# TAMUparametric/PPOPT

Measured on AMD Instinct MI355X. Metric: candidate active-sets checked/sec (combinatorial mpQP), higher is better.
Workload: dtype f64

## Files before the change

ppopt_amd/csrc/batch_level.hip:

```cpp
#define MPC_GLOBAL __device__ __forceinline__
#define MPC_LB(...)
#include "batch_level.hpp"
#include "knobs.hpp"

#include <algorithm>
#include <cmath>
#include <cstdlib>
#include <cstring>
#include <mutex>
#include <tuple>
#include <vector>

namespace mpc {
namespace {

#define MEMBER const BatchMember &m = tab[blockIdx.y]
__device__ __forceinline__ int32_t *part_list_of(const BatchMember &m, int c) { return m.part_lists + (size_t)c * (size_t)m.n; }

__global__ void __launch_bounds__(256) m_zero(const BatchMember *__restrict__ tab) {
    MEMBER;
    for (int z = 0; z < m.n_zero; ++z) {
        const unsigned long long bytes = m.zero[z].bytes;
        if ((reinterpret_cast<unsigned long long>(m.zero[z].p) & 7ull) == 0 && (bytes & 7ull) == 0) {
            unsigned long long *p = reinterpret_cast<unsigned long long *>(m.zero[z].p);
            for (unsigned long long i = blockIdx.x * 256ull + threadIdx.x; i < bytes / 8; i += (unsigned long long)gridDim.x * 256ull) p[i] = 0ull;
        } else {
            unsigned char *p = reinterpret_cast<unsigned char *>(m.zero[z].p);
            for (unsigned long long i = blockIdx.x * 256ull + threadIdx.x; i < bytes; i += (unsigned long long)gridDim.x * 256ull) p[i] = 0;
        }
    }
}
__global__ void m_zero_counter(const BatchMember *__restrict__ tab, int which) {
    MEMBER;
    if (threadIdx.x == 0) { if (which == 0) m.ctr->work_retry = 0u; else m.ctr->work_region = 0u; }
}

template <int K, int NT, int SP>
__global__ void __launch_bounds__(256) m_kkt_thread(const BatchMember *__restrict__ tab) {
    MEMBER;
    k_kkt_thread<K, NT, SP>(m.pf, m.fr, m.n, m.kkt_code, m.kkt_L, m.status, m.targs, m.ctr);
}
__global__ void __launch_bounds__(1024) m_compact_small(const BatchMember *__restrict__ tab, int lo, int hi, int into_retry, int slot) {
    MEMBER;
    k_compact_small(m.status, (int)m.n, lo, hi, into_retry ? m.retry_list : m.theta_list, m.dcnt + slot);
}
template <int NT, int SLOTS>
__global__ void __launch_bounds__(64, (SLOTS >= 2 ? (NT <= 4 ? TH_WAVES_S2 : 2) : (NT >= 8 ? 3 : 4))) m_theta2(const BatchMember *__restrict__ tab) {
    MEMBER;
    ThetaArgs ta = m.targs;
    ta.chunk = 1;
    if (m.th_blocks > 0) { ta.wave_max = m.th_blocks; ta.wave_div = 0; }
    const uint8_t *kkc = nullptr;
    const double *kkl = nullptr;
    const int32_t *list = nullptr;
    if (m.use_kkt) { kkc = m.kkt_code; kkl = m.kkt_L; list = m.theta_list; ta.n_dev = m.dcnt + DC_THETA; }
    k_theta2<NT, SLOTS>(m.pf, m.fr, m.n, m.k, m.status, m.ctr, kkc, kkl, ta, list);
}
__global__ void __launch_bounds__(1024) m_partition_small(const BatchMember *__restrict__ tab, unsigned long long spec, int slot) {
    MEMBER;
    k_partition_small(m.status, (int)m.n, spec, m.part_lists, m.n, m.dcnt + slot);
}
__global__ void __launch_bounds__(64) m_verdict(const BatchMember *__restrict__ tab, int slot) {
    MEMBER;
    k_verdict(m.Pv, m.fr, m.n, m.k, m.status, m.ctr, part_list_of(m, 0), m.dcnt + slot);
}

__global__ void __launch_bounds__(64) m_recession(const BatchMember *__restrict__ tab) {
    MEMBER;
    if (!m.theta_open) return;
    k_recession(m.Pv, m.fr, m.n, m.k, m.status);
}

template <int NT, int SLOTS>
__global__ void __launch_bounds__(64, (SLOTS >= 2 ? 2 : R2W)) m_region2(const BatchMember *__restrict__ tab) {
    MEMBER;
    const uint8_t *kkc = m.use_kkt ? m.kkt_code : nullptr;
    const double *kkl = m.use_kkt ? m.kkt_L : nullptr;
    RegionStream rs = m.rs;
    rs.max_blocks = m.r2_blocks;
    if (m.r2_wcap > 0) rs.w_cap = m.r2_wcap;
    k_region2<NT, SLOTS>(m.pr, m.fr, m.k, part_list_of(m, 2), (int)m.n, m.status, m.headd, m.headi, m.fd, m.fi, m.epool, m.ctr, kkc, kkl, m.W,
                         m.kept_g, m.ldk, m.done_g, m.no_rbox ? (const double *)nullptr : m.targs.tvp + (size_t)NT * NT + NT, rs);
}

template <int MODE>
__global__ void __launch_bounds__(64) m_region_v1(const BatchMember *__restrict__ tab) {
    MEMBER;
    const int n_list = m.dcnt[DC_BATCH_RRETRY];
    if (n_list <= 0 || n_list > m.rcap) return;
    k_region<MODE>(m.Pr, m.fr, m.k, m.retry_list, n_list, m.status, m.recd, m.reci, m.rec_d, m.rec_i, m.ctr, m.facet_flags);
}

template <int SLOTS>
__global__ void __launch_bounds__(64, XQ_WAVES) m_xq(const BatchMember *__restrict__ tab) {
    MEMBER;
    DictCache dq = m.dc;
    dq.n_list_dev = m.dcnt + DC_OPEN;
    dq.max_blocks = m.xq_blocks;
    k_xq<SLOTS>(m.pf, m.fr, m.k, part_list_of(m, 3), (int)m.n, m.status, m.ctr, dq, m.nxc);
}
template <int NXC, int SLOTS>
__global__ void __launch_bounds__(64, (NXC * SLOTS >= 64 ? 2 : (NXC * SLOTS >= 32 ? X2_WAVES : X2_WAVES_16))) m_x2(const BatchMember *__restrict__ tab) {
    MEMBER;
    DictCache d = m.dc;
    d.n_list_dev = m.dcnt + (m.quick_test ? DC_OPEN_QT : DC_OPEN);
    d.max_blocks = m.x2_blocks;
    k_x2<NXC, SLOTS>(m.pf, m.fr, m.k, m.quick_test ? m.retry_list : part_list_of(m, 3), (int)m.n, m.status, m.ctr, d);
}

template <int MW>
__global__ void m_pruned_append(const BatchMember *__restrict__ tab) {
    MEMBER;
    k_pruned_append<MW>(m.fr, m.n, m.k, m.status, m.pruned + (size_t)m.n_pruned * MW, m.ctr, m.keep_lowdim);
}
// ... 209 lines not shown
```

ppopt_amd/csrc/kernels2.hpp:

```cpp
#pragma once
#include <type_traits>
#include "kernels.hpp"
#include "lp_reg.hpp"

namespace mpc {

constexpr double GROWTH_FRESH = 1e6;
#ifndef THETA_SCALE_MODE
#define THETA_SCALE_MODE 0
#endif
__device__ __forceinline__ double theta_row_scale(int ex) {
    if (THETA_SCALE_MODE == 1) return 1.0;
    if (THETA_SCALE_MODE == 2 && ex > 0) return 1.0;
    return ldexp(1.0, -ex);
}


struct ThetaArgs {
    const double *W, *UVp, *tvp, *tv_rows;
    int chunk;
    int cbuf_off;
    const int32_t *n_dev;
    const double *Wr, *UVrp, *AATr, *Me, *Ne, *gE;
    int ne;
// ... 204 lines not shown
            bbase[threadIdx.x] = tot ? atomicAdd(threadIdx.x == 0 ? ta.kt_n : ta.kx_n, tot) : 0;
        }
        __syncthreads();
        if (kind) {
            const int li = kind - 1;
            int pos = bbase[li] + __popcll((li ? m2 : m1) & ((1ull << lane) - 1ull));
            for (int w = 0; w < wave; ++w) pos += wcnt[li][w];
            (li ? ta.kx_list : ta.kt_list)[pos] = (int)c;
        }
    }
}

__device__ inline int kkt_fetch_or_solve(const DevProblem &P, int k, Smem &s, const uint8_t *kkcode, const double *Lin, size_t c,
                                         bool *ill = nullptr) {
    if (kkcode) {
        int code = kkcode[c];
        if (code != KK_UNDECIDED) {
            if (code == KK_ILL) { if (ill) *ill = true; code = 0; }
            if (code == 0) {
                const int cnt = k * (P.n_t + 1);
                const double *src = Lin + c * (size_t)cnt;
                for (int idx = lane_id(); idx < cnt; idx += 64) s.L[idx] = src[idx];
                wave_sync();
            }
            return code;
        }
    }
    return kkt_solve(P, k, s, ill);
}

#ifndef TH_WAVES_S2
#define TH_WAVES_S2 3
#endif
template <int NT, int SLOTS>
MPC_GLOBAL void MPC_LB(64, (SLOTS >= 2 ? (NT <= 4 ? TH_WAVES_S2 : 2) : (NT >= 8 ? 3 : 4))) k_theta2(const DevProblem *__restrict__ Pg, const int32_t *__restrict__ cands, long long n, int k,
                                                    uint8_t *__restrict__ status, LevelCounters *__restrict__ ctr,
                                                    const uint8_t *__restrict__ kkcode, const double *__restrict__ Lin, ThetaArgs ta,
                                                    const int32_t *__restrict__ list) {
    const DevProblem &P = *Pg;
    if (ta.n_dev) {
        n = *ta.n_dev;
        long long active = gridDim.x;
        if (ta.wave_max > 0) active = min(active, (long long)ta.wave_max);
        if (ta.wave_div > 0) active = min(active, max(256ll, n / ta.wave_div));
        if (ta.chunk <= 0) ta.chunk = (int)max(1ll, min(16ll, n / (active * 8)));
        if ((long long)blockIdx.x >= active || (long long)blockIdx.x * ta.chunk >= n) return;
    }
    extern __shared__ __attribute__((aligned(16))) double smem[];
    Smem s = carve(P, smem);
    constexpr int LS = NT + 1;
    const int lane = lane_id(), nt = P.n_t, nr = nt + 1, e = P.n_eq, nc = P.n_c, mode = P.kkt_mode, npre = P.n_tpre;
    double *tvm = s.T, *tvt = s.T + NT * NT, *blo = tvt + NT, *bhi = blo + NT, *Lp = s.T + NT * NT + 3 * NT;
    for (int idx = lane; idx < NT * NT + 3 * NT; idx += 64) s.T[idx] = ta.tvp[idx];
    wave_sync();
    unsigned long long pivots = 0, n_retry = 0;
    long long cyc_kkt = 0, cyc_theta = 0, cyc_rows = 0, cyc_s2 = 0;
    unsigned long long n_box1 = 0, n_box2 = 0;
    for (;;) {
        unsigned int c0 = 0;
        if (lane == 0) c0 = atomicAdd(&ctr->work_verdict, (unsigned)ta.chunk);
        c0 = (unsigned)__builtin_amdgcn_readfirstlane((int)c0);
        if (c0 >= n) break;
        const unsigned c1 = (unsigned)min((long long)c0 + ta.chunk, n);
      for (unsigned w = c0; w < c1; ++w) {
        const unsigned c = list ? (unsigned)list[w] : w;
        const int nin = load_active_set(P, cands + (size_t)c * k, k, s);
        int st = -1;
        const long long t0 = clock64();
        const int kk = kkt_fetch_or_solve(P, k, s, kkcode, Lin, c);
        const long long t1 = clock64();
        cyc_kkt += t1 - t0;
        bool singular = false, retry = false;
        if (kk == 1) st = ST_INFEASIBLE;
        else if (kk == 2) singular = true;
        else if (kk == 0) {
            for (int idx = lane; idx < k * LS; idx += 64) {
                const int a = idx / LS, t = idx - a * LS;
                Lp[idx] = t <= nt ? s.L[a * nr + t] : 0.0;
            }
            wave_sync();
            RegLp<NT + 2, SLOTS, true> lp;
            const int nlam = k - e, m = nlam + nin + npre;
            lp.m = m; lp.iters = 0; lp.max_iter = 50 * (m + nt) + 100; lp.growth = 0.0;
            lp.alive = (nt >= 31 ? 0xfffffffeu : ((1u << (nt + 1)) - 2u));
            lp.cv = nt + m + lane - 1;
            bool box_lam = false, box_slack = false;
            bool live[SLOTS];
#pragma unroll
            for (int sl = 0; sl < SLOTS; ++sl) live[sl] = (lane + 64 * sl) < (k - e) + nin + npre;
#pragma unroll
            for (int sl = 0; sl < SLOTS; ++sl) {
                const int i = lane + 64 * sl;
                double h = 0.0, g[NT];
#pragma unroll
                for (int t = 0; t < NT; ++t) g[t] = 0.0;
                lp.var[sl] = nt + i;
                lp.kind[sl] = i < nlam ? RK_PASSIVE : (i < m ? RK_INEQ : RK_DEAD);
                lp.w[sl] = 1.0; lp.winv[sl] = 1.0;
                bool pre = false;
                if (i < nlam) {
                    h = Lp[(e + i) * LS];
#pragma unroll
                    for (int t = 0; t < NT; ++t) g[t] = -Lp[(e + i) * LS + 1 + t];
                } else if (i < nlam + nin) {
                    const int ci = s.inact[i - nlam];
                    if (mode == 0) {
                        double acc[NT + 1], w[8];
                        const double *Wrow = ta.W + (size_t)ci * nc;
#pragma unroll
                        for (int a = 0; a < 8; ++a) { const int asv = s.as[a]; w[a] = Wrow[a < k ? asv : 0]; }
#pragma unroll
                        for (int t = 0; t <= NT; ++t) acc[t] = ta.UVp[ci * LS + t];
#pragma unroll
                        for (int a = 0; a < 8; ++a) {
// ... 103 lines not shown
                else if (r1 == LP_OPTIMAL && inf2) st = ST_FEASIBLE;
                else if (r1 == LP_OPTIMAL) {
#pragma unroll
                    for (int sl = 0; sl < S; ++sl) if (q.kind[sl] == RK_PASSIVE) q.kind[sl] = RK_INEQ;
                    const int r2 = q.phase1();
                    if (r2 == LP_ITERLIMIT) st = ST_LP_LIMIT;
                    else if (q.growth > GROWTH_FRESH) retry = true;
                    else st = r2 == LP_OPTIMAL ? ST_OPT_PENDING : ST_FEASIBLE;
                }
                lp_iters = q.iters;
            };
            bool compacted = false;
            if constexpr (SLOTS == 2) {
                const unsigned long long b0 = __ballot(live[0]), b1 = __ballot(live[1]);
                const int n_live = __popcll(b0) + __popcll(b1);
                if (ta.cbuf_off > 0 && n_live <= 64 && !inf1) {
                    constexpr int CS = NT + 4;
                    double *cb = smem + ta.cbuf_off;
                    int *cbi = reinterpret_cast<int *>(cb + 64 * CS);
                    const unsigned long long below = (1ull << lane) - 1ull;
#pragma unroll
                    for (int sl = 0; sl < 2; ++sl) {
                        if (live[sl]) {
                            const int pos = sl == 0 ? __popcll(b0 & below) : __popcll(b0) + __popcll(b1 & below);
#pragma unroll
                            for (int j = 0; j < NT + 2; ++j) cb[pos * CS + j] = lp.t[sl][j];
                            cb[pos * CS + NT + 2] = lp.w[sl];
                            cb[pos * CS + NT + 3] = lp.winv[sl];
                            cbi[2 * pos] = lp.var[sl];
                            cbi[2 * pos + 1] = lp.kind[sl];
                        }
                    }
                    wave_sync();
                    RegLp<NT + 2, 1, true> lp1;
                    lp1.m = n_live; lp1.iters = 0; lp1.max_iter = lp.max_iter; lp1.growth = 0.0;
                    lp1.alive = lp.alive; lp1.cv = lp.cv;
                    const bool has = lane < n_live;
#pragma unroll
                    for (int j = 0; j < NT + 2; ++j) lp1.t[0][j] = has ? cb[lane * CS + j] : 0.0;
                    lp1.w[0] = has ? cb[lane * CS + NT + 2] : 1.0;
                    lp1.winv[0] = has ? cb[lane * CS + NT + 3] : 1.0;
                    lp1.var[0] = has ? cbi[2 * lane] : -1;
                    lp1.kind[0] = has ? cbi[2 * lane + 1] : RK_DEAD;
                    wave_sync();
                    stages(lp1, std::integral_constant<int, 1>{});
                    compacted = true;
                }
            }
            if (!compacted) stages(lp, std::integral_constant<int, SLOTS>{});
            pivots += lp_iters;
            cyc_s2 += clock64() - t15;
        }
        const long long t2 = clock64();
        cyc_theta += t2 - t1;
        if (st < 0 && !retry) st = singular ? ST_NEEDX_SING : ST_NEEDX;
        if (retry) { st = ST_RETRY; n_retry++; }
        if (lane == 0) status[c] = (uint8_t)st;
      }
    }
    if (lane == 0) {
        atomicAdd(&ctr->cycles[0], (unsigned long long)cyc_kkt); atomicAdd(&ctr->cycles[1], (unsigned long long)cyc_theta);
        atomicAdd(&ctr->cycles[4], (unsigned long long)cyc_rows); atomicAdd(&ctr->cycles[5], (unsigned long long)cyc_s2);
        atomicAdd(&ctr->cycles[6], n_box1); atomicAdd(&ctr->cycles[7], n_box2); atomicAdd(&ctr->n_retry_theta, (unsigned)n_retry);
        atomicAdd(&ctr->pivots, pivots); atomicAdd(&ctr->xtheta_fallbacks, n_retry);
    }
}

// ... 834 lines not shown
                if (lane == 0) { om[2 * sl] = (int)(unsigned)bm; om[2 * sl + 1] = (int)(unsigned)(bm >> 32); }
            }
#pragma unroll
            for (int sl = 0; sl < SLOTS; ++sl) {
                const int i = lane + 64 * sl, cidx = var[sl] - nv;
                if (i < mr && cidx >= 0 && cidx < ncp) opos[cidx] = (uint8_t)i;
            }
            { const int cidx = cvv - nv; if (lane >= 1 && lane <= nc0 && ((alive >> lane) & 1u) && cidx >= 0 && cidx < ncp) opos[cidx] = (uint8_t)(128 + lane); }
        }
        if (lane == 0) {
            oi[2 * mr + NXC] = (int)alive;
            oi[2 * mr + NXC + 1] = __double2hiint(growth);
            oi[2 * mr + NXC + 2] = __double2loint(growth);
            dc.stored[c] = 1;
        }
        cur = nxt;
    }
    if (ctr && lane == 0 && pivots) atomicAdd(&ctr->pivots, pivots);
}

typedef const __attribute__((address_space(1))) double *gdp;
constexpr double BOX_REDUNDANT_MARGIN = 1e-6;

struct RegionStream {
    unsigned int *count;
    int32_t *flags;
    int shift;
    int n_slots;
    const int32_t *n_opt_dev;
    int w_cap, w_max;
    int max_blocks;
};

template <int NT, int SLOTS>
MPC_GLOBAL void MPC_LB(64, (SLOTS >= 2 ? 2 : R2W)) k_region2(
    const DevProblem *__restrict__ Pg, const int32_t *__restrict__ cands, int k, const int32_t *__restrict__ opt_list, int n_opt,
    uint8_t *__restrict__ status, double *__restrict__ head_d, int32_t *__restrict__ head_i, int fd, int fi,
    double *__restrict__ epool, LevelCounters *__restrict__ ctr, const uint8_t *__restrict__ kkcode, const double *__restrict__ Lin,
    int W, uint8_t *__restrict__ kept_g, int ldk, unsigned int *__restrict__ done_g, const double *__restrict__ box, RegionStream rs) {
    const DevProblem &P = *Pg;
    extern __shared__ __attribute__((aligned(16))) double smem[];
    Smem s = carve(P, smem);
    const int lane = lane_id(), nt = P.n_t, nr = nt + 1, nx = P.n_x, nc = P.n_c, ntc = P.n_tc, e = P.n_eq;
    constexpr int NC = NT + 3;
    constexpr int ID_SIGMA = 4096, ID_R = 8192;
    unsigned long long pivots = 0;
    long long cyc = 0, rc_rows = 0, rc_cheb = 0, rc_facet = 0, rc_tot = 0, rc_refac = 0, rc_fpiv = 0, rc_box = 0;
    if (rs.n_opt_dev) {
        n_opt = *rs.n_opt_dev;
        if (W == 0) { W = rs.w_max > 0 ? rs.w_max : 1; while (W > 1 && (long long)n_opt * W > rs.w_cap) W >>= 1; }
        if ((long long)blockIdx.x >= (long long)n_opt * W || (rs.max_blocks > 0 && (int)blockIdx.x >= rs.max_blocks)) return;
    }
    if (lane == 0) atomicMax(&ctr->r2_not_t0, ~(unsigned long long)wall_clock64());
    double *tvm = s.T, *tvt = s.T + NT * NT, *blo = tvt + NT, *bhi = blo + NT;
    { gdp src = (gdp)P.tvp; for (int idx = lane; idx < NT * NT + 3 * NT; idx += 64) s.T[idx] = src[idx]; }
    wave_sync();
    for (;;) {
        unsigned int item = 0;
        if (lane == 0) item = atomicAdd(&ctr->work_r2, 1u);
        item = (unsigned)__builtin_amdgcn_readfirstlane((int)item);
        if (item >= (unsigned)n_opt * (unsigned)W) break;
        const unsigned int w = item / (unsigned)W;
        const int part = (int)(item - w * (unsigned)W);
        auto own = [&](int row) -> bool { return W == 1 || row % W == part; };
        bool is_last = true;
        const long long t0 = clock64();
        const int c = opt_list[w];
// ... 32 lines not shown
                    for (int u = 0; u < 4; ++u) {
                        const int idx = idx0 + 64 * u, ic = idx < nxr ? idx : 0;
                        ii[u] = ic / nr; tt[u] = ic - ii[u] * nr;
                        acc[u] = X0H[ic];
                    }
                    int a = 0;
                    for (; a + 4 <= k; a += 4) {
                        double gv[4][4];
#pragma unroll
                        for (int v = 0; v < 4; ++v) {
                            const int ra = s.as[a + v] * nx;
#pragma unroll
                            for (int u = 0; u < 4; ++u) gv[v][u] = Gt[ra + ii[u]];
                        }
#pragma unroll
                        for (int v = 0; v < 4; ++v)
#pragma unroll
                            for (int u = 0; u < 4; ++u) acc[u] = fma(-gv[v][u], s.L[(a + v) * nr + tt[u]], acc[u]);
                    }
                    for (; a < k; ++a) {
                        const int ra = s.as[a] * nx;
                        double gv[4];
#pragma unroll
                        for (int u = 0; u < 4; ++u) gv[u] = Gt[ra + ii[u]];
#pragma unroll
                        for (int u = 0; u < 4; ++u) acc[u] = fma(-gv[u], s.L[a * nr + tt[u]], acc[u]);
                    }
#pragma unroll
                    for (int u = 0; u < 4; ++u) if (idx0 + 64 * u < nxr) s.X[idx0 + 64 * u] = acc[u];
                }
                wave_sync();
            }
            const int nlam = k - e, m = nlam + nin + ntc, ldE = nr;
            RegLp<NC, SLOTS> lp;
            lp.m = m + 1; lp.iters = 0; lp.max_iter = 50 * (m + nt) + 200; lp.growth = 0.0;
            lp.alive = (1u << (nt + 2)) - 2u;
            lp.cv = lane <= nt ? ID_SIGMA + lane : ID_R;
            wave_sync();
            auto build_rows = [&](auto FULLC) {
                constexpr bool FULL = decltype(FULLC)::value;
                gdp gb = (gdp)P.b, gF = (gdp)P.F, gbt = (gdp)P.b_t, gAt = (gdp)P.A_t, gAT = (gdp)P.AT;
#pragma unroll
                for (int sl = 0; sl < SLOTS; ++sl) {
                    const int i = lane + 64 * sl;
                    double h = 0.0, g[NT];
#pragma unroll
                    for (int t = 0; t < NT; ++t) g[t] = 0.0;
                    const bool is_lam = i < nlam, is_in = !is_lam && i < nlam + nin, is_tc = !is_lam && !is_in && i < m;
                    const int ci = is_in ? s.inact[i - nlam] : 0, it = is_tc ? i - nlam - nin : 0;
                    double hv = 0.0, fv[NT];
#pragma unroll
                    for (int t = 0; t < NT; ++t) fv[t] = 0.0;
                    if (is_in || is_tc) {
                        gdp hp = is_in ? gb + ci : gbt + it;
                        gdp fp = is_in ? gF + (size_t)ci * nt : gAt + (size_t)it * nt;
                        hv = *hp;
#pragma unroll
                        for (int t = 0; t < NT; ++t) if (FULL || t < nt) fv[t] = fp[t];
                    }
                    if (is_lam) {
                        h = s.L[(e + i) * nr];
#pragma unroll
                        for (int t = 0; t < NT; ++t) if (FULL || t < nt) g[t] = -s.L[(e + i) * nr + 1 + t];
                    } else if (is_in) {
                        gdp at = gAT + ci;
                        double acc[NT + 1];
#pragma unroll
// ... 111 lines not shown
                    const int i = lane + 64 * sl;
                    if (i < m && s.kept[i] != 3) {
                        double sl_i = s.E[i * ldE];
#pragma unroll
                        for (int t = 0; t < NT; ++t) if (t < nt) sl_i = fma(-s.E[i * ldE + 1 + t], th[t], sl_i);
                        rv = fmin(rv, sl_i);
                    }
                }
                rv = dpp_wave_min(rv);
                if (!(r1 == LP_OPTIMAL && r2 != 2 && rv > 2 * FULL_DIM_RADIUS)) { retry = true; reason = 1; }
            }
            else if (r1 != LP_OPTIMAL || r2 == 2 || !(radius > FULL_DIM_RADIUS)) st = ST_OPT_NO_REGION;
            const long long tr2 = clock64();
            rc_cheb += tr2 - tr1;
            const int it_cheb = lp.iters;
            if (st == ST_REGION && !retry) {
                lp.set_kind(m, RK_DEAD);
                int rz = LP_OPTIMAL;
                if (rrow >= 0) rz = lp.drive_to_zero(rrow);
                else {
                    const unsigned long long bc = __ballot(lp.cv == ID_R && lane >= 1 && lane < NC && ((lp.alive >> lane) & 1u));
                    if (bc) lp.drop_col(__ffsll((long long)bc) - 1);
                }
                if (rz != LP_OPTIMAL) { retry = true; reason = 2; }
                constexpr double KEEP_TOL = TOL_FEAS;
                auto mark_tight = [&]() {
                    if (lane >= 1 && lane < NC && ((lp.alive >> lane) & 1u) && lp.cv < m && own(lp.cv)) s.kept[lp.cv] = 1;
#pragma unroll
                    for (int sl = 0; sl < SLOTS; ++sl)
                        if (lp.kind[sl] == RK_INEQ && lp.var[sl] < m && lp.t[sl][0] <= KEEP_TOL && own(lp.var[sl])) s.kept[lp.var[sl]] = 1;
#pragma unroll
                    for (int sl = 0; sl < SLOTS; ++sl) {
                        if (lp.kind[sl] == RK_INEQ && lp.var[sl] < m && lp.t[sl][0] > KEEP_TOL && own(lp.var[sl])) {
                            double mx = 0.0;
#pragma unroll
                            for (int j = 1; j < NC; ++j) mx = bare_max(mx, (double)lp.t[sl][j]);
                            if (R2_CERT && !(mx > TOL_COST) && s.kept[lp.var[sl]] == 0) {
                                s.kept[lp.var[sl]] = 2;
#ifdef R2_DEBUG
                                printf("row %d: certificate at a final vertex, beta=%.3e mx=%.3e\n", lp.var[sl], (double)lp.t[sl][0], mx);
#endif
                            }
                        }
                    }
                    wave_sync();
                };
                auto mark_vertex = [&]() {
                    if (lp.growth > GROWTH_SAFE) return;
                    if (lane >= 1 && lane < NC && ((lp.alive >> lane) & 1u) && lp.cv < m && own(lp.cv)) s.kept[lp.cv] = 1;
#pragma unroll
                    for (int sl = 0; sl < SLOTS; ++sl) {
                        if (lp.kind[sl] == RK_INEQ && lp.var[sl] < m && own(lp.var[sl])) {
                            if (lp.t[sl][0] <= KEEP_TOL) s.kept[lp.var[sl]] = 1;
                            else {
                                double mx = 0.0;
#pragma unroll
                                for (int j = 1; j < NC; ++j) mx = bare_max(mx, (double)lp.t[sl][j]);
                                if (R2_CERT && !(mx > TOL_COST) && s.kept[lp.var[sl]] == 0) {
                                    s.kept[lp.var[sl]] = 2;
#ifdef R2_DEBUG
                                    printf("row %d: certificate at an intermediate vertex, beta=%.3e mx=%.3e\n", lp.var[sl], (double)lp.t[sl][0], mx);
#endif
                                }
                            }
                        }
                    }
                };
                auto row_of = [&](int id, double &h, double (&g)[NT]) {
#pragma unroll
                    for (int t = 0; t < NT; ++t) g[t] = 0.0;
                    h = 0.0;
                    if (id < m) {
                        h = s.E[id * ldE];
#pragma unroll
                        for (int t = 0; t < NT; ++t) if (t < nt) g[t] = s.E[id * ldE + 1 + t];
                    } else if (id > ID_SIGMA && id <= ID_SIGMA + nt) {
                        const int tr = P.tv_tight[id - ID_SIGMA - 1];
                        h = P.b_t[tr];
#pragma unroll
                        for (int t = 0; t < NT; ++t) if (t < nt) g[t] = P.A_t[tr * nt + t];
                    }
                };
                auto refactor = [&]() -> bool {
                    const unsigned al = (unsigned)uni((int)lp.alive);
                    if (__popc(al) != nt) return false;
                    rc_refac++;
                    double *Bm = s.K, *R = s.K + nt * nt;
                    wave_sync();
                    if (lane >= 1 && lane < NC && ((al >> lane) & 1u)) {
                        const int c = __popc(al & ((1u << lane) - 1u));
// ... 18 lines not shown
                        for (int t = 0; t < NT; ++t) if (t < nt) b0 = fma(-g[t], R[t * (nt + 1)], b0);
                        lp.t[sl][0] = live ? b0 : 0.0;
                        if (live && b0 < -10 * TOL_FEAS) ok = false;
#pragma unroll
                        for (int j = 1; j < NC; ++j) {
                            double acc = 0.0;
                            if (j <= nt) {
#pragma unroll
                                for (int t = 0; t < NT; ++t) if (t < nt) acc = fma(g[t], R[t * (nt + 1) + j], acc);
                            }
                            lp.t[sl][j] = live ? -acc : 0.0;
                        }
                    }
                    lp.cv = (lane >= 1 && lane <= nt) ? s.colvar[lane - 1] : -1;
                    lp.alive = (1u << (nt + 1)) - 2u;
                    lp.growth = 0.0;
                    wave_sync();
                    return !__any(!ok);
                };
                if (!retry && lp.growth > GROWTH_SAFE && !refactor()) { retry = true; reason = 3; }
                if (!retry) mark_tight();
                int refactors = 0;
                bool retested = false;
                for (int cidx = 0; cidx < m && !retry && st == ST_REGION; ++cidx) {
                    if (s.kept[cidx] != 0 || !own(cidx)) continue;
                    int row = -1;
#pragma unroll
                    for (int sl = SLOTS - 1; sl >= 0; --sl) {
                        const unsigned long long br = __ballot(lp.var[sl] == cidx && lp.kind[sl] == RK_INEQ);
                        if (br) row = __ffsll((long long)br) - 1 + 64 * sl;
                    }
                    if (row < 0) { retry = true; reason = 4; break; }
                    lp.set_kind(row, RK_X0);
                    const int pr = lp.primal_hook(row, -1, false, false, mark_vertex);
                    if (pr == 3) { st = ST_LP_LIMIT; break; }
                    bool kept_c = pr == 4;
                    if (pr != 4) { kept_c = lp.beta(row) <= KEEP_TOL; lp.set_kind(row, RK_INEQ); }
                    bool rebuild = false;
                    if (lp.growth > GROWTH_SAFE) {
                        const bool clear_cut = kept_c || lp.beta(row) > 1e3 * TOL_FEAS;
                        if (!retested || lp.growth > 1e6 || !clear_cut) {
                            if (retested || ++refactors > 64 || !refactor()) { retry = true; reason = retested ? 5 : 6; break; }
                            mark_tight();
                            retested = true;
                            --cidx;
                            continue;
                        }
                        lp.growth = 0.0;
                    }
                    retested = false;
                    wave_sync();
#ifdef R2_DEBUG
                    if (lane == 0) printf("row %d: LP pr=%d beta=%.3e growth=%.3e kept=%d iters=%d\n", cidx, pr, lp.beta(row), lp.growth, (int)kept_c, lp.iters);
#endif
                    if (lane == 0) s.kept[cidx] = kept_c ? 1 : 2;
                    wave_sync();
                    if (rebuild && (++refactors > 64 || !refactor())) { retry = true; reason = 6; break; }
                    mark_tight();
                }
            }
            pivots += lp.iters;
            const long long tr3 = clock64();
            rc_facet += tr3 - tr2;
            rc_fpiv += lp.iters - it_cheb;
            if (W > 1) {
                for (int i = lane; i < m; i += 64) if (own(i)) kept_g[(size_t)w * ldk + i] = (uint8_t)s.kept[i];
                const unsigned fb = (retry ? 1u : 0u) | (st == ST_LP_LIMIT ? 2u : 0u);
// ... 139 lines not shown
```

ppopt_amd/csrc/lp_reg.hpp:

```cpp
#pragma once
#include "lp_engine.hpp"

namespace mpc {

constexpr int RK_COST = 7;

__device__ __forceinline__ int uni(int v) { return __builtin_amdgcn_readfirstlane(v); }

__device__ __forceinline__ double readlane_f64(double v, int lane) {
    const int lo = __builtin_amdgcn_readlane(__double2loint(v), lane);
    const int hi = __builtin_amdgcn_readlane(__double2hiint(v), lane);
    return __hiloint2double(hi, lo);
}

template <int CTRL> __device__ __forceinline__ int dpp_i32(int v) { return __builtin_amdgcn_update_dpp(v, v, CTRL, 0xf, 0xf, false); }
template <int CTRL> __device__ __forceinline__ double dpp_f64(double v) {
    return __hiloint2double(dpp_i32<CTRL>(__double2hiint(v)), dpp_i32<CTRL>(__double2loint(v)));
}
template <int CTRL> __device__ __forceinline__ int dpp_all_i32(int v) { return __builtin_amdgcn_update_dpp(0, v, CTRL, 0xf, 0xf, true); }
template <int CTRL> __device__ __forceinline__ double dpp_all_f64(double v) {
    return __hiloint2double(dpp_all_i32<CTRL>(__double2hiint(v)), dpp_all_i32<CTRL>(__double2loint(v)));
}
__device__ __forceinline__ double bare_min(double a, double b) { double r; asm("v_min_f64 %0, %1, %2" : "=v"(r) : "v"(a), "v"(b)); return r; }
__device__ __forceinline__ double bare_max(double a, double b) { double r; asm("v_max_f64 %0, %1, %2" : "=v"(r) : "v"(a), "v"(b)); return r; }
__device__ __forceinline__ double bare_min_s(double a_uniform, double b) { double r; asm("v_min_f64 %0, %1, %2" : "=v"(r) : "s"(a_uniform), "v"(b)); return r; }
__device__ __forceinline__ double bare_max_s(double a_uniform, double b) { double r; asm("v_max_f64 %0, %1, %2" : "=v"(r) : "s"(a_uniform), "v"(b)); return r; }
__device__ __forceinline__ float bare_maxf(float a, float b) { float r; asm("v_max_f32 %0, %1, %2" : "=v"(r) : "v"(a), "v"(b)); return r; }
__device__ __forceinline__ float bare_maxf_s(float a_uniform, float b) { float r; asm("v_max_f32 %0, %1, %2" : "=v"(r) : "s"(a_uniform), "v"(b)); return r; }
__device__ __forceinline__ double rot_wave_min(double v) {
    v = bare_min(v, dpp_all_f64<0x121>(v)); v = bare_min(v, dpp_all_f64<0x122>(v)); v = bare_min(v, dpp_all_f64<0x124>(v)); v = bare_min(v, dpp_all_f64<0x128>(v));
    const double a = readlane_f64(v, 0), b = readlane_f64(v, 16), c = readlane_f64(v, 32), d = readlane_f64(v, 48);
    return bare_min_s(d, bare_min_s(c, bare_min_s(b, bare_min_s(a, v))));
}
__device__ __forceinline__ double rot_wave_max(double v) {
    v = bare_max(v, dpp_all_f64<0x121>(v)); v = bare_max(v, dpp_all_f64<0x122>(v)); v = bare_max(v, dpp_all_f64<0x124>(v)); v = bare_max(v, dpp_all_f64<0x128>(v));
    const double a = readlane_f64(v, 0), b = readlane_f64(v, 16), c = readlane_f64(v, 32), d = readlane_f64(v, 48);
    return bare_max_s(d, bare_max_s(c, bare_max_s(b, bare_max_s(a, v))));
}
__device__ __forceinline__ double dpp_wave_min(double v) {
    v = fmin(v, dpp_f64<0x111>(v)); v = fmin(v, dpp_f64<0x112>(v)); v = fmin(v, dpp_f64<0x114>(v)); v = fmin(v, dpp_f64<0x118>(v));
    return fmin(fmin(readlane_f64(v, 15), readlane_f64(v, 31)), fmin(readlane_f64(v, 47), readlane_f64(v, 63)));
}
__device__ __forceinline__ double dpp_wave_max(double v) {
    v = fmax(v, dpp_f64<0x111>(v)); v = fmax(v, dpp_f64<0x112>(v)); v = fmax(v, dpp_f64<0x114>(v)); v = fmax(v, dpp_f64<0x118>(v));
    return fmax(fmax(readlane_f64(v, 15), readlane_f64(v, 31)), fmax(readlane_f64(v, 47), readlane_f64(v, 63)));
}
__device__ __forceinline__ bool key_better(unsigned long long ok, int oi, unsigned long long k, int i) {
    return oi >= 0 && (i < 0 || ok > k || (ok == k && oi < i));
}
template <int CTRL> __device__ __forceinline__ void argmax_step(unsigned long long &key, int &idx) {
    const unsigned lo = (unsigned)dpp_i32<CTRL>((int)(unsigned)key), hi = (unsigned)dpp_i32<CTRL>((int)(unsigned)(key >> 32));
    const int oi = dpp_i32<CTRL>(idx);
    const unsigned long long ok = ((unsigned long long)hi << 32) | lo;
    if (key_better(ok, oi, key, idx)) { key = ok; idx = oi; }
}
__device__ __forceinline__ int dpp_wave_argmax(unsigned long long key, int idx) {
    argmax_step<0x111>(key, idx); argmax_step<0x112>(key, idx); argmax_step<0x114>(key, idx); argmax_step<0x118>(key, idx);
    unsigned long long bk = 0; int bi = -1;
#pragma unroll
    for (int l = 15; l < 64; l += 16) {
        const unsigned lo = (unsigned)__builtin_amdgcn_readlane((int)(unsigned)key, l), hi = (unsigned)__builtin_amdgcn_readlane((int)(unsigned)(key >> 32), l);
        const int oi = __builtin_amdgcn_readlane(idx, l);
        const unsigned long long ok = ((unsigned long long)hi << 32) | lo;
        if (key_better(ok, oi, bk, bi)) { bk = ok; bi = oi; }
    }
    return bi;
}
__device__ __forceinline__ unsigned long long f64_key(double v) {
    const unsigned long long b = (unsigned long long)__double_as_longlong(v);
    return (b & 0x8000000000000000ull) ? ~b : (b | 0x8000000000000000ull);
}

__device__ __forceinline__ double fast_rcp(double x) {
    double r = __builtin_amdgcn_rcp(x);
    double e = fma(-x, r, 1.0);
    r = fma(r, e, r);
    e = fma(-x, r, 1.0);
    return fma(r, e, r);
}
__device__ __forceinline__ float dpp_wave_max_f32(float v) {
    v = fmaxf(v, __int_as_float(dpp_i32<0x111>(__float_as_int(v)))); v = fmaxf(v, __int_as_float(dpp_i32<0x112>(__float_as_int(v))));
    v = fmaxf(v, __int_as_float(dpp_i32<0x114>(__float_as_int(v)))); v = fmaxf(v, __int_as_float(dpp_i32<0x118>(__float_as_int(v))));
    const int b = __float_as_int(v);
    return fmaxf(fmaxf(__int_as_float(__builtin_amdgcn_readlane(b, 15)), __int_as_float(__builtin_amdgcn_readlane(b, 31))),
                 fmaxf(__int_as_float(__builtin_amdgcn_readlane(b, 47)), __int_as_float(__builtin_amdgcn_readlane(b, 63))));
}
__device__ __forceinline__ float rot_wave_max_f32(float v) {
    v = bare_maxf(v, __int_as_float(dpp_all_i32<0x121>(__float_as_int(v)))); v = bare_maxf(v, __int_as_float(dpp_all_i32<0x122>(__float_as_int(v))));
    v = bare_maxf(v, __int_as_float(dpp_all_i32<0x124>(__float_as_int(v)))); v = bare_maxf(v, __int_as_float(dpp_all_i32<0x128>(__float_as_int(v))));
    const int b = __float_as_int(v);
    const float r0 = __int_as_float(__builtin_amdgcn_readlane(b, 0)), r1 = __int_as_float(__builtin_amdgcn_readlane(b, 16));
    const float r2 = __int_as_float(__builtin_amdgcn_readlane(b, 32)), r3 = __int_as_float(__builtin_amdgcn_readlane(b, 48));
    return bare_maxf_s(r3, bare_maxf_s(r2, bare_maxf_s(r1, bare_maxf_s(r0, v))));
}
__device__ __forceinline__ int dpp_wave_min_i32(int v) {
    v = min(v, dpp_i32<0x111>(v)); v = min(v, dpp_i32<0x112>(v)); v = min(v, dpp_i32<0x114>(v)); v = min(v, dpp_i32<0x118>(v));
    return min(min(__builtin_amdgcn_readlane(v, 15), __builtin_amdgcn_readlane(v, 31)), min(__builtin_amdgcn_readlane(v, 47), __builtin_amdgcn_readlane(v, 63)));
}

__device__ __forceinline__ double opaque(double e) { asm volatile("" : "+v"(e)); return e; }
__device__ __forceinline__ int opaque(int e) { asm volatile("" : "+v"(e)); return e; }

template <int W> struct RowVec;
template <> struct RowVec<8> { typedef double type __attribute__((ext_vector_type(8))); };
template <> struct RowVec<16> { typedef double type __attribute__((ext_vector_type(16))); };

template <int NC, bool SELECT = false>
struct RegRow {
    static constexpr int W = NC <= 8 ? 8 : 16;
    static constexpr int H = (NC + W - 1) / W;
    static_assert(H <= 2, "at most 32 columns");
    typename RowVec<W>::type v[H];
    __device__ __forceinline__ double get(int j) const { return v[j / W][j % W]; }
    __device__ __forceinline__ void set(int j, double x) { v[j / W][j % W] = x; }
    __device__ __forceinline__ double getq(int q) const {
        if (H == 1) return v[0][q];
        return q < W ? v[0][q] : v[H - 1][q - W];
    }
    __device__ __forceinline__ void setq(int q, double x) {
        if (H == 1) v[0][q] = x;
        else if (q < W) v[0][q] = x;
        else v[H - 1][q - W] = x;
// ... 2 lines not shown
        RegRow &row; int j;
        __device__ __forceinline__ operator double() const { return row.get(j); }
        __device__ __forceinline__ Ref &operator=(double x) { row.set(j, x); return *this; }
    };
    __device__ __forceinline__ Ref operator[](int j) { return Ref{*this, j}; }
    __device__ __forceinline__ double operator[](int j) const { return get(j); }
};

template <int NC>
struct RegRow<NC, true> {
    double v[NC];
    __device__ __forceinline__ double get(int j) const { return v[j]; }
    __device__ __forceinline__ void set(int j, double x) { v[j] = x; }
    static __device__ __forceinline__ double in_register(double e) { return opaque(e); }
    __device__ __forceinline__ double getq(int q) const {
        double r = in_register(v[0]);
#pragma unroll
        for (int j = 1; j < NC; ++j) r = (j == q) ? in_register(v[j]) : r;
        return r;
    }
    __device__ __forceinline__ void setq(int q, double x) {
#pragma unroll
        for (int j = 0; j < NC; ++j) v[j] = (j == q) ? x : in_register(v[j]);
    }
    struct Ref {
        RegRow &row; int j;
        __device__ __forceinline__ operator double() const { return row.get(j); }
        __device__ __forceinline__ Ref &operator=(double x) { row.set(j, x); return *this; }
    };
    __device__ __forceinline__ Ref operator[](int j) { return Ref{*this, j}; }
    __device__ __forceinline__ double operator[](int j) const { return get(j); }
};

template <int NC, int SLOTS, bool WEIGHTED = false>
struct RegLp {
    RegRow<NC, (SLOTS >= 2)> t[SLOTS];
    double w[SLOTS], winv[SLOTS];
    int kind[SLOTS];
    int var[SLOTS];
    int cv;
    unsigned alive;
    int m;
    int iters, max_iter;
    double growth;
    static constexpr bool ROT = !(SLOTS >= 2 && NC > 16);
    static __device__ __forceinline__ double wred_min(double v) { return ROT ? rot_wave_min(v) : dpp_wave_min(v); }
    static __device__ __forceinline__ double wred_max(double v) { return ROT ? rot_wave_max(v) : dpp_wave_max(v); }
    static __device__ __forceinline__ float wred_max_f32(float v) { return ROT ? rot_wave_max_f32(v) : dpp_wave_max_f32(v); }

    __device__ __forceinline__ double row_entry(int r, const double (&c)[SLOTS]) const {
        const int rl = r & 63;
        if (SLOTS == 1) return readlane_f64(c[0], rl);
        return readlane_f64((r >> 6) ? opaque(c[SLOTS - 1]) : opaque(c[0]), rl);
    }
    __device__ __forceinline__ int row_entry_i(int r, const int (&c)[SLOTS]) const {
        const int rl = r & 63;
        if (SLOTS == 1) return __builtin_amdgcn_readlane(c[0], rl);
        return __builtin_amdgcn_readlane((r >> 6) ? opaque(c[SLOTS - 1]) : opaque(c[0]), rl);
    }

    __device__ __forceinline__ void pivot_core(int r, int q, const double (&f)[SLOTS], double inv) {
        const int lane = lane_id();
        double fz[SLOTS];
#pragma unroll
        for (int s = 0; s < SLOTS; ++s) {
            const bool is_r = (lane + 64 * s) == r;
            t[s].setq(q, is_r ? 1.0 : 0.0);
            fz[s] = is_r ? 0.0 : f[s];
            if (is_r) {
#pragma unroll
                for (int j = 0; j < NC; ++j) t[s].set(j, t[s].get(j) * inv);
            }
        }
        if (SLOTS == 1) {
#pragma unroll
            for (int j = 0; j < NC; ++j) {
                const double trj = readlane_f64(t[0].get(j), r & 63);
#pragma unroll
                for (int s = 0; s < SLOTS; ++s) t[s].set(j, fma(-fz[s], trj, t[s].get(j)));
            }
        } else {
// ... 26 lines not shown
#pragma unroll
        for (int s = 0; s < SLOTS; ++s) t[s].setq(q, 0.0);
    }

    __device__ __forceinline__ void set_kind(int r, int k) {
        const int lane = lane_id();
#pragma unroll
        for (int s = 0; s < SLOTS; ++s) if ((lane + 64 * s) == r) kind[s] = k;
    }
    __device__ __forceinline__ int get_kind(int r) const { return row_entry_i(r, kind); }
    __device__ __forceinline__ double beta(int r) const {
        double c0[SLOTS];
#pragma unroll
        for (int s = 0; s < SLOTS; ++s) c0[s] = t[s].get(0);
        return row_entry(r, c0);
    }

    __device__ __forceinline__ int best_col(int r_in) const {
        const int r = uni(r_in);
        int q[SLOTS];
#pragma unroll
        for (int s = 0; s < SLOTS; ++s) {
            q[s] = -1;
            double best = TOL_PIV;
#pragma unroll
            for (int j = 1; j < NC; ++j) {
                const double a = fabs(t[s].get(j));
                if (a > best) { best = a; q[s] = j; }
            }
        }
        return row_entry_i(r, q);
    }

    template <bool P1>
    __device__ __forceinline__ int price(int crow) const {
        int q[SLOTS];
#pragma unroll
        for (int s = 0; s < SLOTS; ++s) {
            double best = P1 ? TOL_COST : -TOL_COST;
#pragma unroll
            for (int j = 1; j < NC; ++j) best = P1 ? bare_max(best, t[s].get(j)) : bare_min(best, t[s].get(j));
            q[s] = -1;
#pragma unroll
            for (int j = NC - 1; j >= 1; --j) q[s] = (t[s].get(j) == best) ? j : q[s];
            if (!(P1 ? best > TOL_COST : best < -TOL_COST)) q[s] = -1;
        }
        return row_entry_i(crow, q);
    }
    template <bool P1>
    __device__ __forceinline__ unsigned improving_mask(int crow) const {
        int mk[SLOTS];
#pragma unroll
        for (int s = 0; s < SLOTS; ++s) {
            mk[s] = 0;
#pragma unroll
            for (int j = 1; j < NC; ++j) {
                const double g = P1 ? t[s].get(j) : -t[s].get(j);
                if (g > TOL_COST) mk[s] |= (1 << j);
            }
        }
        return (unsigned)row_entry_i(crow, mk);
    }

    struct NoHook { __device__ __forceinline__ void operator()() const {} };
    __device__ __forceinline__ int primal(int phase1_row, int cost_row, bool drop_on_leave = true, bool decide_only = false) {
        return primal_hook(phase1_row, cost_row, drop_on_leave, decide_only, NoHook());
    }
    template <class Hook>
    __device__ __forceinline__ int primal_hook(int phase1_row, int cost_row, bool drop_on_leave, bool decide_only, Hook after_pivot) {
        const int lane = lane_id();
        int deg = 0;
        for (;;) {
            if (iters > max_iter) return 3;
            const bool bland = deg > DEG_SWITCH;
            const int crow = uni(phase1_row >= 0 ? phase1_row : cost_row);
            if (phase1_row >= 0 && beta(phase1_row) <= TOL_FEAS) return 0;
            int q = phase1_row >= 0 ? price<true>(crow) : price<false>(crow);
            if (q < 0) return 0;
            if (bland) {
                const unsigned improving = phase1_row >= 0 ? improving_mask<true>(crow) : improving_mask<false>(crow);
                const bool mine = lane >= 1 && lane < NC && ((improving >> lane) & 1u);
                const int vmin = dpp_wave_min_i32(mine ? cv : 0x7fffffff);
                q = __ffsll((long long)__ballot(mine && cv == vmin)) - 1;
            }
            q = uni(q);
            double a[SLOTS], ratio[SLOTS];
            bool elig[SLOTS];
            float cmf = 0.0f;
            double tmax = INFINITY;
#pragma unroll
            for (int s = 0; s < SLOTS; ++s) {
                const int i = lane + 64 * s;
                a[s] = t[s].getq(q);
                const bool used = (i < m) & (kind[s] != RK_DEAD);
                if (used) cmf = fmaxf(cmf, fabsf((float)a[s]));
                elig[s] = used & ((kind[s] == RK_INEQ) | (kind[s] == RK_X0)) & (a[s] > TOL_PIV);
                const double b0 = fmax(t[s].get(0), 0.0), ia = fast_rcp(elig[s] ? a[s] : 1.0);
                ratio[s] = elig[s] ? b0 * ia : 0.0;
                tmax = fmin(tmax, elig[s] ? (b0 + HARRIS_DELTA) * ia : INFINITY);
            }
            const float colmax = wred_max_f32(cmf);
            tmax = wred_min(tmax);
            if (tmax == INFINITY) return 2;
            int r = -1;
            bool leaving_x0 = false;
            double rpiv = 0.0;
            if (bland) {
                double rm = INFINITY;
#pragma unroll
                for (int s = 0; s < SLOTS; ++s) if (elig[s]) rm = fmin(rm, ratio[s]);
                rm = wred_min(rm);
                unsigned long long key = 0; int idx = -1;
#pragma unroll
                for (int s = 0; s < SLOTS; ++s)
                    if (elig[s] && ratio[s] == rm) {
                        const unsigned long long kk = ((unsigned long long)(kind[s] == RK_X0) << 40) | (unsigned long long)(0x7fffffff - var[s]);
                        if (key_better(kk, lane + 64 * s, key, idx)) { key = kk; idx = lane + 64 * s; }
                    }
                r = dpp_wave_argmax(key, idx);
                if (r < 0) return 2;
                rpiv = row_entry(r, a);
                leaving_x0 = get_kind(r) == RK_X0;
            } else {
                bool pass[SLOTS];
#pragma unroll
                for (int s = 0; s < SLOTS; ++s) pass[s] = elig[s] && !(ratio[s] > tmax);
#pragma unroll
                for (int s = SLOTS - 1; s >= 0; --s) {
                    const unsigned long long bx = __ballot(pass[s] && kind[s] == RK_X0);
                    if (bx) { r = __ffsll((long long)bx) - 1 + 64 * s; leaving_x0 = true; }
                }
                if (leaving_x0) rpiv = row_entry(r, a);
                else {
                    double am = 0.0;
#pragma unroll
                    for (int s = 0; s < SLOTS; ++s) if (pass[s]) am = fmax(am, a[s]);
                    rpiv = wred_max(am);
#pragma unroll
                    for (int s = SLOTS - 1; s >= 0; --s) {
                        const unsigned long long br = __ballot(pass[s] && a[s] == rpiv);
                        if (br) r = __ffsll((long long)br) - 1 + 64 * s;
                    }
                    if (r < 0) return 2;
                }
            }
            r = uni(r);
            const double rmin = row_entry(r, ratio), inv = fast_rcp(rpiv);
            growth = fmax(growth, (double)(colmax * (float)inv));
            deg = (rmin <= 0.0) ? deg + 1 : 0;
            const bool skip = leaving_x0 && decide_only;
            if (!skip) { pivot_core(r, q, a, inv); after_pivot(); }
            else iters++;
            if (leaving_x0) { set_kind(r, RK_INEQ); if (drop_on_leave && !skip) drop_col(q); return 4; }
        }
    }

    __device__ __forceinline__ int drive_to_zero(int r, bool decide_only = false) {
        set_kind(r, RK_X0);
        const int st = primal(r, -1, true, decide_only);
        if (st == 3) return LP_ITERLIMIT;
        if (st != 4) {
            if (beta(r) > TOL_FEAS) return LP_INFEASIBLE;
            if (decide_only) return LP_OPTIMAL;
            const int qq = best_col(r);
            if (qq < 0) set_kind(r, RK_DEAD);
            else { pivot(r, qq); set_kind(r, RK_INEQ); drop_col(qq); }
        }
        return LP_OPTIMAL;
    }

    __device__ __forceinline__ int phase1() {
        const int lane = lane_id();
        bool neg[SLOTS];
        double vmin = INFINITY;
#pragma unroll
        for (int s = 0; s < SLOTS; ++s) {
            const double v0 = WEIGHTED ? t[s].get(0) * winv[s] : t[s].get(0);
            neg[s] = lane + 64 * s < m && kind[s] == RK_INEQ && v0 < -TOL_FEAS;
            if (neg[s]) vmin = fmin(vmin, v0);
        }
        vmin = wred_min(vmin);
        if (vmin == INFINITY) return LP_OPTIMAL;
        int r = -1;
#pragma unroll
// ... 19 lines not shown
```

Measured before the change: 325.4 million.

## Slim register-LP inner loop: tree reductions, reused reciprocal, DPP broadcast, fused vertex hook

Measured after the change: 329.3 million (median of 3 runs). No clear change (+1.2%).

```diff
diff --git a/ppopt_amd/csrc/batch_level.hip b/ppopt_amd/csrc/batch_level.hip
--- a/ppopt_amd/csrc/batch_level.hip
+++ b/ppopt_amd/csrc/batch_level.hip
@@ -54,7 +54,7 @@
     const double *kkl = nullptr;
     const int32_t *list = nullptr;
     if (m.use_kkt) { kkc = m.kkt_code; kkl = m.kkt_L; list = m.theta_list; ta.n_dev = m.dcnt + DC_THETA; }
-    k_theta2<NT, SLOTS>(m.pf, m.fr, m.n, m.k, m.status, m.ctr, kkc, kkl, ta, list);
+    k_theta2<NT, SLOTS, false>(m.pf, m.fr, m.n, m.k, m.status, m.ctr, kkc, kkl, ta, list);
 }
 __global__ void __launch_bounds__(1024) m_partition_small(const BatchMember *__restrict__ tab, unsigned long long spec, int slot) {
     MEMBER;
@@ -79,7 +79,7 @@
     RegionStream rs = m.rs;
     rs.max_blocks = m.r2_blocks;
     if (m.r2_wcap > 0) rs.w_cap = m.r2_wcap;
-    k_region2<NT, SLOTS>(m.pr, m.fr, m.k, part_list_of(m, 2), (int)m.n, m.status, m.headd, m.headi, m.fd, m.fi, m.epool, m.ctr, kkc, kkl, m.W,
+    k_region2<NT, SLOTS, (SLOTS < 2)>(m.pr, m.fr, m.k, part_list_of(m, 2), (int)m.n, m.status, m.headd, m.headi, m.fd, m.fi, m.epool, m.ctr, kkc, kkl, m.W,
                          m.kept_g, m.ldk, m.done_g, m.no_rbox ? (const double *)nullptr : m.targs.tvp + (size_t)NT * NT + NT, rs);
 }
 
diff --git a/ppopt_amd/csrc/kernels2.hpp b/ppopt_amd/csrc/kernels2.hpp
--- a/ppopt_amd/csrc/kernels2.hpp
+++ b/ppopt_amd/csrc/kernels2.hpp
@@ -260,11 +260,12 @@
 #ifndef TH_WAVES_S2
 #define TH_WAVES_S2 3
 #endif
-template <int NT, int SLOTS>
+template <int NT, int SLOTS, bool DIET = true>
 MPC_GLOBAL void MPC_LB(64, (SLOTS >= 2 ? (NT <= 4 ? TH_WAVES_S2 : 2) : (NT >= 8 ? 3 : 4))) k_theta2(const DevProblem *__restrict__ Pg, const int32_t *__restrict__ cands, long long n, int k,
                                                     uint8_t *__restrict__ status, LevelCounters *__restrict__ ctr,
                                                     const uint8_t *__restrict__ kkcode, const double *__restrict__ Lin, ThetaArgs ta,
                                                     const int32_t *__restrict__ list) {
+    constexpr bool LP_DIET = DIET && !(SLOTS >= 2 && NT > 8);
     const DevProblem &P = *Pg;
     if (ta.n_dev) {
         n = *ta.n_dev;
@@ -307,7 +308,7 @@
                 Lp[idx] = t <= nt ? s.L[a * nr + t] : 0.0;
             }
             wave_sync();
-            RegLp<NT + 2, SLOTS, true> lp;
+            RegLp<NT + 2, SLOTS, true, LP_DIET> lp;
             const int nlam = k - e, m = nlam + nin + npre;
             lp.m = m; lp.iters = 0; lp.max_iter = 50 * (m + nt) + 100; lp.growth = 0.0;
             lp.alive = (nt >= 31 ? 0xfffffffeu : ((1u << (nt + 1)) - 2u));
@@ -477,7 +478,7 @@
                         }
                     }
                     wave_sync();
-                    RegLp<NT + 2, 1, true> lp1;
+                    RegLp<NT + 2, 1, true, LP_DIET> lp1;
                     lp1.m = n_live; lp1.iters = 0; lp1.max_iter = lp.max_iter; lp1.growth = 0.0;
                     lp1.alive = lp.alive; lp1.cv = lp.cv;
                     const bool has = lane < n_live;
@@ -1378,7 +1379,7 @@
     int max_blocks;
 };
 
-template <int NT, int SLOTS>
+template <int NT, int SLOTS, bool DIET = true>
 MPC_GLOBAL void MPC_LB(64, (SLOTS >= 2 ? 2 : R2W)) k_region2(
     const DevProblem *__restrict__ Pg, const int32_t *__restrict__ cands, int k, const int32_t *__restrict__ opt_list, int n_opt,
     uint8_t *__restrict__ status, double *__restrict__ head_d, int32_t *__restrict__ head_i, int fd, int fi,
@@ -1477,7 +1478,7 @@
                 wave_sync();
             }
             const int nlam = k - e, m = nlam + nin + ntc, ldE = nr;
-            RegLp<NC, SLOTS> lp;
+            RegLp<NC, SLOTS, false, DIET> lp;
             lp.m = m + 1; lp.iters = 0; lp.max_iter = 50 * (m + nt) + 200; lp.growth = 0.0;
             lp.alive = (1u << (nt + 2)) - 2u;
             lp.cv = lane <= nt ? ID_SIGMA + lane : ID_R;
@@ -1655,9 +1656,7 @@
 #pragma unroll
                     for (int sl = 0; sl < SLOTS; ++sl) {
                         if (lp.kind[sl] == RK_INEQ && lp.var[sl] < m && lp.t[sl][0] > KEEP_TOL && own(lp.var[sl])) {
-                            double mx = 0.0;
-#pragma unroll
-                            for (int j = 1; j < NC; ++j) mx = bare_max(mx, (double)lp.t[sl][j]);
+                            const double mx = lp.row_max(sl, 0.0);
                             if (R2_CERT && !(mx > TOL_COST) && s.kept[lp.var[sl]] == 0) {
                                 s.kept[lp.var[sl]] = 2;
 #ifdef R2_DEBUG
@@ -1668,7 +1667,7 @@
                     }
                     wave_sync();
                 };
-                auto mark_vertex = [&]() {
+                auto mark_vertex = [&](const double (&rowmax)[SLOTS]) {
                     if (lp.growth > GROWTH_SAFE) return;
                     if (lane >= 1 && lane < NC && ((lp.alive >> lane) & 1u) && lp.cv < m && own(lp.cv)) s.kept[lp.cv] = 1;
 #pragma unroll
@@ -1676,9 +1675,7 @@
                         if (lp.kind[sl] == RK_INEQ && lp.var[sl] < m && own(lp.var[sl])) {
                             if (lp.t[sl][0] <= KEEP_TOL) s.kept[lp.var[sl]] = 1;
                             else {
-                                double mx = 0.0;
-#pragma unroll
-                                for (int j = 1; j < NC; ++j) mx = bare_max(mx, (double)lp.t[sl][j]);
+                                const double mx = DIET ? rowmax[sl] : lp.row_max(sl, 0.0);
                                 if (R2_CERT && !(mx > TOL_COST) && s.kept[lp.var[sl]] == 0) {
                                     s.kept[lp.var[sl]] = 2;
 #ifdef R2_DEBUG
@@ -1763,7 +1760,7 @@
                     }
                     if (row < 0) { retry = true; reason = 4; break; }
                     lp.set_kind(row, RK_X0);
-                    const int pr = lp.primal_hook(row, -1, false, false, mark_vertex);
+                    const int pr = lp.template primal_hook<DIET>(row, -1, false, false, mark_vertex);
                     if (pr == 3) { st = ST_LP_LIMIT; break; }
                     bool kept_c = pr == 4;
                     if (pr != 4) { kept_c = lp.beta(row) <= KEEP_TOL; lp.set_kind(row, RK_INEQ); }
diff --git a/ppopt_amd/csrc/lp_reg.hpp b/ppopt_amd/csrc/lp_reg.hpp
--- a/ppopt_amd/csrc/lp_reg.hpp
+++ b/ppopt_amd/csrc/lp_reg.hpp
@@ -27,13 +27,25 @@
 __device__ __forceinline__ double bare_max_s(double a_uniform, double b) { double r; asm("v_max_f64 %0, %1, %2" : "=v"(r) : "s"(a_uniform), "v"(b)); return r; }
 __device__ __forceinline__ float bare_maxf(float a, float b) { float r; asm("v_max_f32 %0, %1, %2" : "=v"(r) : "v"(a), "v"(b)); return r; }
 __device__ __forceinline__ float bare_maxf_s(float a_uniform, float b) { float r; asm("v_max_f32 %0, %1, %2" : "=v"(r) : "s"(a_uniform), "v"(b)); return r; }
-__device__ __forceinline__ double rot_wave_min(double v) {
+template <int CTRL, int ROWS> __device__ __forceinline__ int dpp_rows_i32(int v) { return __builtin_amdgcn_mov_dpp(v, CTRL, ROWS, 0xf, false); }
+template <int CTRL, int ROWS> __device__ __forceinline__ double dpp_rows_f64(double v) {
+    return __hiloint2double(dpp_rows_i32<CTRL, ROWS>(__double2hiint(v)), dpp_rows_i32<CTRL, ROWS>(__double2loint(v)));
+}
+template <bool BC> __device__ __forceinline__ double rot_wave_min(double v) {
     v = bare_min(v, dpp_all_f64<0x121>(v)); v = bare_min(v, dpp_all_f64<0x122>(v)); v = bare_min(v, dpp_all_f64<0x124>(v)); v = bare_min(v, dpp_all_f64<0x128>(v));
+    if (BC) {
+        v = bare_min(v, dpp_rows_f64<0x142, 0xa>(v)); v = bare_min(v, dpp_rows_f64<0x143, 0xc>(v));
+        return readlane_f64(v, 63);
+    }
     const double a = readlane_f64(v, 0), b = readlane_f64(v, 16), c = readlane_f64(v, 32), d = readlane_f64(v, 48);
     return bare_min_s(d, bare_min_s(c, bare_min_s(b, bare_min_s(a, v))));
 }
-__device__ __forceinline__ double rot_wave_max(double v) {
+template <bool BC> __device__ __forceinline__ double rot_wave_max(double v) {
     v = bare_max(v, dpp_all_f64<0x121>(v)); v = bare_max(v, dpp_all_f64<0x122>(v)); v = bare_max(v, dpp_all_f64<0x124>(v)); v = bare_max(v, dpp_all_f64<0x128>(v));
+    if (BC) {
+        v = bare_max(v, dpp_rows_f64<0x142, 0xa>(v)); v = bare_max(v, dpp_rows_f64<0x143, 0xc>(v));
+        return readlane_f64(v, 63);
+    }
     const double a = readlane_f64(v, 0), b = readlane_f64(v, 16), c = readlane_f64(v, 32), d = readlane_f64(v, 48);
     return bare_max_s(d, bare_max_s(c, bare_max_s(b, bare_max_s(a, v))));
 }
@@ -85,9 +97,13 @@
     return fmaxf(fmaxf(__int_as_float(__builtin_amdgcn_readlane(b, 15)), __int_as_float(__builtin_amdgcn_readlane(b, 31))),
                  fmaxf(__int_as_float(__builtin_amdgcn_readlane(b, 47)), __int_as_float(__builtin_amdgcn_readlane(b, 63))));
 }
-__device__ __forceinline__ float rot_wave_max_f32(float v) {
+template <bool BC> __device__ __forceinline__ float rot_wave_max_f32(float v) {
     v = bare_maxf(v, __int_as_float(dpp_all_i32<0x121>(__float_as_int(v)))); v = bare_maxf(v, __int_as_float(dpp_all_i32<0x122>(__float_as_int(v))));
     v = bare_maxf(v, __int_as_float(dpp_all_i32<0x124>(__float_as_int(v)))); v = bare_maxf(v, __int_as_float(dpp_all_i32<0x128>(__float_as_int(v))));
+    if (BC) {
+        v = bare_maxf(v, __int_as_float(dpp_rows_i32<0x142, 0xa>(__float_as_int(v)))); v = bare_maxf(v, __int_as_float(dpp_rows_i32<0x143, 0xc>(__float_as_int(v))));
+        return __int_as_float(__builtin_amdgcn_readlane(__float_as_int(v), 63));
+    }
     const int b = __float_as_int(v);
     const float r0 = __int_as_float(__builtin_amdgcn_readlane(b, 0)), r1 = __int_as_float(__builtin_amdgcn_readlane(b, 16));
     const float r2 = __int_as_float(__builtin_amdgcn_readlane(b, 32)), r3 = __int_as_float(__builtin_amdgcn_readlane(b, 48));
@@ -156,7 +172,17 @@
     __device__ __forceinline__ double operator[](int j) const { return get(j); }
 };
 
-template <int NC, int SLOTS, bool WEIGHTED = false>
+template <bool MAX, int LO, int HI, class Row>
+__device__ __forceinline__ double row_tree(const Row &row, double leaf0) {
+    if constexpr (HI - LO == 1) return LO == 0 ? leaf0 : (double)row.get(LO);
+    else {
+        constexpr int MID = (LO + HI) / 2;
+        const double a = row_tree<MAX, LO, MID>(row, leaf0), b = row_tree<MAX, MID, HI>(row, leaf0);
+        return MAX ? bare_max(a, b) : bare_min(a, b);
+    }
+}
+
+template <int NC, int SLOTS, bool WEIGHTED = false, bool DIET = true>
 struct RegLp {
     RegRow<NC, (SLOTS >= 2)> t[SLOTS];
     double w[SLOTS], winv[SLOTS];
@@ -168,9 +194,12 @@
     int iters, max_iter;
     double growth;
     static constexpr bool ROT = !(SLOTS >= 2 && NC > 16);
-    static __device__ __forceinline__ double wred_min(double v) { return ROT ? rot_wave_min(v) : dpp_wave_min(v); }
-    static __device__ __forceinline__ double wred_max(double v) { return ROT ? rot_wave_max(v) : dpp_wave_max(v); }
-    static __device__ __forceinline__ float wred_max_f32(float v) { return ROT ? rot_wave_max_f32(v) : dpp_wave_max_f32(v); }
+    static constexpr bool TREE = ROT && DIET;
+    static constexpr bool ONE_RCP = ROT && DIET;
+    static constexpr bool BCAST = ROT && DIET;
+    static __device__ __forceinline__ double wred_min(double v) { return ROT ? rot_wave_min<BCAST>(v) : dpp_wave_min(v); }
+    static __device__ __forceinline__ double wred_max(double v) { return ROT ? rot_wave_max<BCAST>(v) : dpp_wave_max(v); }
+    static __device__ __forceinline__ float wred_max_f32(float v) { return ROT ? rot_wave_max_f32<BCAST>(v) : dpp_wave_max_f32(v); }
 
     __device__ __forceinline__ double row_entry(int r, const double (&c)[SLOTS]) const {
         const int rl = r & 63;
@@ -263,18 +292,30 @@
         return row_entry_i(r, q);
     }
 
+    __device__ __forceinline__ double row_max(int s, double floor) const {
+        if (TREE) return row_tree<true, 0, NC>(t[s], floor);
+        double b = floor;
+#pragma unroll
+        for (int j = 1; j < NC; ++j) b = bare_max(b, t[s].get(j));
+        return b;
+    }
+
     template <bool P1>
-    __device__ __forceinline__ int price(int crow) const {
+    __device__ __forceinline__ int price(int crow, double (&best)[SLOTS]) const {
         int q[SLOTS];
 #pragma unroll
         for (int s = 0; s < SLOTS; ++s) {
-            double best = P1 ? TOL_COST : -TOL_COST;
-#pragma unroll
-            for (int j = 1; j < NC; ++j) best = P1 ? bare_max(best, t[s].get(j)) : bare_min(best, t[s].get(j));
+            double b = P1 ? TOL_COST : -TOL_COST;
+            if (TREE) b = row_tree<P1, 0, NC>(t[s], b);
+            else {
+#pragma unroll
+                for (int j = 1; j < NC; ++j) b = P1 ? bare_max(b, t[s].get(j)) : bare_min(b, t[s].get(j));
+            }
             q[s] = -1;
 #pragma unroll
-            for (int j = NC - 1; j >= 1; --j) q[s] = (t[s].get(j) == best) ? j : q[s];
-            if (!(P1 ? best > TOL_COST : best < -TOL_COST)) q[s] = -1;
+            for (int j = NC - 1; j >= 1; --j) q[s] = (t[s].get(j) == b) ? j : q[s];
+            if (!(P1 ? b > TOL_COST : b < -TOL_COST)) q[s] = -1;
+            best[s] = b;
         }
         return row_entry_i(crow, q);
     }
@@ -293,21 +334,24 @@
         return (unsigned)row_entry_i(crow, mk);
     }
 
-    struct NoHook { __device__ __forceinline__ void operator()() const {} };
+    struct NoHook { __device__ __forceinline__ void operator()(const double (&)[SLOTS]) const {} };
     __device__ __forceinline__ int primal(int phase1_row, int cost_row, bool drop_on_leave = true, bool decide_only = false) {
         return primal_hook(phase1_row, cost_row, drop_on_leave, decide_only, NoHook());
     }
-    template <class Hook>
-    __device__ __forceinline__ int primal_hook(int phase1_row, int cost_row, bool drop_on_leave, bool decide_only, Hook after_pivot) {
+    template <bool AT_TOP = true, class Hook>
+    __device__ __forceinline__ int primal_hook(int phase1_row, int cost_row, bool drop_on_leave, bool decide_only, Hook at_vertex) {
         const int lane = lane_id();
         int deg = 0;
+        bool moved = false;
         for (;;) {
             if (iters > max_iter) return 3;
             const bool bland = deg > DEG_SWITCH;
             const int crow = uni(phase1_row >= 0 ? phase1_row : cost_row);
             if (phase1_row >= 0 && beta(phase1_row) <= TOL_FEAS) return 0;
-            int q = phase1_row >= 0 ? price<true>(crow) : price<false>(crow);
+            double best[SLOTS];
+            int q = phase1_row >= 0 ? price<true>(crow, best) : price<false>(crow, best);
             if (q < 0) return 0;
+            if (AT_TOP && moved) at_vertex(best);
             if (bland) {
                 const unsigned improving = phase1_row >= 0 ? improving_mask<true>(crow) : improving_mask<false>(crow);
                 const bool mine = lane >= 1 && lane < NC && ((improving >> lane) & 1u);
@@ -315,7 +359,7 @@
                 q = __ffsll((long long)__ballot(mine && cv == vmin)) - 1;
             }
             q = uni(q);
-            double a[SLOTS], ratio[SLOTS];
+            double a[SLOTS], ratio[SLOTS], ia[SLOTS];
             bool elig[SLOTS];
             float cmf = 0.0f;
             double tmax = INFINITY;
@@ -326,9 +370,10 @@
                 const bool used = (i < m) & (kind[s] != RK_DEAD);
                 if (used) cmf = fmaxf(cmf, fabsf((float)a[s]));
                 elig[s] = used & ((kind[s] == RK_INEQ) | (kind[s] == RK_X0)) & (a[s] > TOL_PIV);
-                const double b0 = fmax(t[s].get(0), 0.0), ia = fast_rcp(elig[s] ? a[s] : 1.0);
-                ratio[s] = elig[s] ? b0 * ia : 0.0;
-                tmax = fmin(tmax, elig[s] ? (b0 + HARRIS_DELTA) * ia : INFINITY);
+                const double b0 = fmax(t[s].get(0), 0.0);
+                ia[s] = fast_rcp(elig[s] ? a[s] : 1.0);
+                ratio[s] = elig[s] ? b0 * ia[s] : 0.0;
+                tmax = fmin(tmax, elig[s] ? (b0 + HARRIS_DELTA) * ia[s] : INFINITY);
             }
             const float colmax = wred_max_f32(cmf);
             tmax = wred_min(tmax);
@@ -376,11 +421,11 @@
                 }
             }
             r = uni(r);
-            const double rmin = row_entry(r, ratio), inv = fast_rcp(rpiv);
+            const double rmin = row_entry(r, ratio), inv = ONE_RCP ? row_entry(r, ia) : fast_rcp(rpiv);
             growth = fmax(growth, (double)(colmax * (float)inv));
             deg = (rmin <= 0.0) ? deg + 1 : 0;
             const bool skip = leaving_x0 && decide_only;
-            if (!skip) { pivot_core(r, q, a, inv); after_pivot(); }
+            if (!skip) { pivot_core(r, q, a, inv); moved = true; if (!AT_TOP) at_vertex(best); }
             else iters++;
             if (leaving_x0) { set_kind(r, RK_INEQ); if (drop_on_leave && !skip) drop_col(q); return 4; }
         }
```
